# QZ1-boy/FCVSR

Hardware: AMD Instinct MI355X
Metric: SR frames/sec (7-frame window, 4x 180x320->720x1280) + PSNR vs ref (higher is better)
Workload: dtype bf16

## Files before the change

fcvsr_amd/csrc/feat_extract.hip:

```cpp
#include <type_traits>
#include "common.h"
#include "mfma_util.h"
#include "u8.h"

namespace fcvsr {

constexpr int kFePix = 128;
constexpr int kFeK = 64;
constexpr int kFeLD = kFeK + 8;
constexpr int kFeERow = 64 + 4;
constexpr int kFeMaxBlk = 16;

struct FeatArgs {
  View x;
  const float* tab;
  int B, H, W, cin;
  const uint16_t* w;
  const float* bias;
  int n_blk;
  void* dst[kFeMaxBlk];
  long long dsx[kFeMaxBlk];
  int dch[kFeMaxBlk];
};

template <bool DSTBF, int CIN, int SRC = kSrcF32>
__global__ __launch_bounds__(256, 3) void feat_extract_kernel(FeatArgs a) {
  extern __shared__ __align__(16) unsigned char lds[];
  uint16_t* A_s = reinterpret_cast<uint16_t*>(lds);
  const int tid = threadIdx.x;
  const int lane = tid & 63, wave = tid >> 6;
  const int r = lane & 31, h = lane >> 5;
  float* E_s = reinterpret_cast<float*>(lds + kFePix * kFeLD * 2) + wave * (32 * kFeERow);
  const long long npix = (long long)a.B * a.H * a.W;
  const long long flat0 = (long long)blockIdx.x * kFePix;
  float* tab_s = reinterpret_cast<float*>(lds + kFePix * kFeLD * 2);
  static_assert((kPeak10 + 1) * 4 <= 4 * 32 * kFeERow * 4, "the table must fit into the epilogue tile");
  if constexpr (SRC == kSrcU8) {
    tab_s[tid] = a.tab[tid];
    __syncthreads();
  } else if constexpr (SRC == kSrcU16) {
    reinterpret_cast<float4*>(tab_s)[tid] = reinterpret_cast<const float4*>(a.tab)[tid];
    __syncthreads();
  }

  {
    const int pl = tid & (kFePix - 1), half = tid >> 7;
    const long long p = flat0 + pl;
    const bool pok = p < npix;
    const long long pc = pok ? p : npix - 1;
    const int xx = (int)(pc % a.W);
    const int yy = (int)((pc / a.W) % a.H);
    const int b = (int)(pc / ((long long)a.W * a.H));
    const float* xb = a.x.p + (long long)b * a.x.sb;
    const uint8_t* xb8 = reinterpret_cast<const uint8_t*>(a.x.p) + (long long)b * a.x.sb;
    const uint16_t* xb16 = reinterpret_cast<const uint16_t*>(a.x.p) + (long long)b * a.x.sb;
    const int sy = (int)a.x.sy, sx = (int)a.x.sx, sc = (int)a.x.sc;
    float f[32];
    auto gather = [&](auto koff) {
      constexpr int K0 = decltype(koff)::value;
#pragma unroll
      for (int j = 0; j < 32; ++j) {
        constexpr int dummy = 0; (void)dummy;
        const int k = K0 + j;
        const int tap = k / CIN, c = k - tap * CIN;
        const int iy = yy + tap / 3 - 1, ix = xx + tap % 3 - 1;
        const bool in = pok && k < 9 * CIN && iy >= 0 && iy < a.H && ix >= 0 && ix < a.W;
        const int iyc = iy < 0 ? 0 : (iy > a.H - 1 ? a.H - 1 : iy), ixc = ix < 0 ? 0 : (ix > a.W - 1 ? a.W - 1 : ix);
        const int off = iyc * sy + ixc * sx + (k < 9 * CIN ? c : 0) * sc;
        float v;
        if constexpr (SRC == kSrcU8) v = tab_s[xb8[off]];
        else if constexpr (SRC == kSrcU16) v = sample_value<kPeak10>(tab_s, xb16[off]);
        else v = xb[off];
        f[j] = in ? v : 0.f;
      }
    };
    if (half == 0) gather(std::integral_constant<int, 0>{});
    else gather(std::integral_constant<int, 32>{});
    uint4* d = reinterpret_cast<uint4*>(A_s + pl * kFeLD + half * 32);
#pragma unroll
    for (int q = 0; q < 4; ++q) {
      typedef __attribute__((ext_vector_type(8))) _Float16 h8;
      const h8 pk = {(_Float16)f[8 * q], (_Float16)f[8 * q + 1], (_Float16)f[8 * q + 2], (_Float16)f[8 * q + 3],
                     (_Float16)f[8 * q + 4], (_Float16)f[8 * q + 5], (_Float16)f[8 * q + 6], (_Float16)f[8 * q + 7]};
      d[q] = __builtin_bit_cast(uint4, pk);
    }
  }
  __syncthreads();

  uint4 pf[4];
#pragma unroll
  for (int kk = 0; kk < 4; ++kk) pf[kk] = *reinterpret_cast<const uint4*>(A_s + (wave * 32 + r) * kFeLD + kk * 16 + h * 8);

  uint4 wf[2][4];
#define FCVSR_FE_LOADW(BLK)                                                                                   \
  _Pragma("unroll") for (int nf = 0; nf < 2; ++nf) _Pragma("unroll") for (int kk = 0; kk < 4; ++kk)             \
      wf[nf][kk] = *reinterpret_cast<const uint4*>(a.w + ((long long)(BLK) * 64 + nf * 32 + r) * kFeK + kk * 16 + h * 8)
  FCVSR_FE_LOADW(0);
  const int co = lane & 7, psub = lane >> 3;
  for (int blk = 0; blk < a.n_blk; ++blk) {
    f32x16_t acc[2];
#pragma unroll
    for (int nf = 0; nf < 2; ++nf) {
#pragma unroll
      for (int i = 0; i < 16; ++i) acc[nf][i] = 0.f;
#pragma unroll
      for (int kk = 0; kk < 4; ++kk) acc[nf] = mfma<false>(wf[nf][kk], pf[kk], acc[nf]);
    }
    if (blk + 1 < a.n_blk) FCVSR_FE_LOADW(blk + 1);
#pragma unroll
    for (int nf = 0; nf < 2; ++nf)
#pragma unroll
      for (int g = 0; g < 4; ++g)
        *reinterpret_cast<float4*>(E_s + r * kFeERow + nf * 32 + 8 * g + 4 * h) =
            make_float4(acc[nf][4 * g], acc[nf][4 * g + 1], acc[nf][4 * g + 2], acc[nf][4 * g + 3]);
    __builtin_amdgcn_wave_barrier();
    float4 b0 = make_float4(0.f, 0.f, 0.f, 0.f), b1 = b0;
    if (a.bias) {
      b0 = *reinterpret_cast<const float4*>(a.bias + blk * 64 + co * 8);
      b1 = *reinterpret_cast<const float4*>(a.bias + blk * 64 + co * 8 + 4);
    }
    uint16_t* dp = reinterpret_cast<uint16_t*>(a.dst[blk]) + a.dch[blk] + co * 8;
    const long long dsx = a.dsx[blk];
#pragma unroll
    for (int j = 0; j < 4; ++j) {
      const int pl = j * 8 + psub;
      const long long p = flat0 + wave * 32 + pl;
      if (p < npix) {
        const float* es = E_s + pl * kFeERow + co * 8;
        const float4 e0 = *reinterpret_cast<const float4*>(es), e1 = *reinterpret_cast<const float4*>(es + 4);
        const float4 x0 = make_float4(e0.x + b0.x, e0.y + b0.y, e0.z + b0.z, e0.w + b0.w);
        const float4 x1 = make_float4(e1.x + b1.x, e1.y + b1.y, e1.z + b1.z, e1.w + b1.w);
        const uint2 lo = cvt4<DSTBF>(x0), hi = cvt4<DSTBF>(x1);
        *reinterpret_cast<uint4*>(dp + p * dsx) = make_uint4(lo.x, lo.y, hi.x, hi.y);
      }
    }
    __builtin_amdgcn_wave_barrier();
  }
#undef FCVSR_FE_LOADW
}

}

using namespace fcvsr;

template <int SRC>
static int feat_extract_launch(const fcvsr_view* x, const float* tab, int B, int H, int W, const void* w, const float* bias, int n_blk,
                               void* const* dst, const int64_t* dst_pix_stride, const int32_t* dst_ch_off, int dst_dtype, void* stream) {
  FCVSR_CHECK_ARG((long long)H * x->sy < (1ll << 31) && 7ll * x->sc < (1ll << 31), "image too large for 32-bit offsets");
  FCVSR_CHECK_ARG(B > 0 && H > 0 && W > 0 && n_blk >= 1 && n_blk <= kFeMaxBlk, "bad sizes");
  FCVSR_CHECK_ARG(dst_dtype == FCVSR_BF16 || dst_dtype == FCVSR_F16, "16-bit destinations");
  FCVSR_CHECK_ARG(((uintptr_t)w % 16) == 0 && (bias == nullptr || ((uintptr_t)bias % 16) == 0), "weights / bias 16-byte aligned");
  FeatArgs a;
  a.x = to_view(*x); a.tab = tab; a.B = B; a.H = H; a.W = W; a.cin = x->c;
  a.w = (const uint16_t*)w; a.bias = bias; a.n_blk = n_blk;

  for (int i = 0; i < kFeMaxBlk; ++i) {
    const int s = i < n_blk ? i : 0;
    FCVSR_CHECK_ARG(dst[s] && ((uintptr_t)dst[s] % 16) == 0 && dst_pix_stride[s] % 8 == 0 && dst_ch_off[s] % 8 == 0 &&
                        dst_ch_off[s] >= 0, "destinations: 16-byte aligned, strides / offsets multiples of 8");
    a.dst[i] = dst[s]; a.dsx[i] = dst_pix_stride[s]; a.dch[i] = dst_ch_off[s];
  }
  const size_t lds = (size_t)kFePix * kFeLD * 2 + 4ull * 32 * kFeERow * 4;
  static DevOnce attr;
  {
    hipError_t e = once_per_device(attr, [&] {
      hipError_t e1 = hipFuncSetAttribute((const void*)feat_extract_kernel<true, 7, SRC>, hipFuncAttributeMaxDynamicSharedMemorySize, (int)lds);
      if (e1 == hipSuccess)
        e1 = hipFuncSetAttribute((const void*)feat_extract_kernel<false, 7, SRC>, hipFuncAttributeMaxDynamicSharedMemorySize, (int)lds);
      return e1;
    });
    if (e != hipSuccess) {
      set_error("fcvsr_feat_extract: %s", hipGetErrorString(e));
      return (int)e;
    }
  }
  const long long npix = (long long)B * H * W;
  dim3 grid(cdiv(npix, kFePix));
  hipStream_t st = (hipStream_t)stream;
  if (dst_dtype == FCVSR_BF16) hipLaunchKernelGGL((feat_extract_kernel<true, 7, SRC>), grid, dim3(256), lds, st, a);
  else hipLaunchKernelGGL((feat_extract_kernel<false, 7, SRC>), grid, dim3(256), lds, st, a);
  FCVSR_LAUNCH_CHECK();
  return 0;
}

extern "C" int fcvsr_feat_extract(const fcvsr_view* x, int B, int H, int W, const void* w, const float* bias, int n_blk,
                                  void* const* dst, const int64_t* dst_pix_stride, const int32_t* dst_ch_off, int dst_dtype,
                                  void* stream) {
  FCVSR_CHECK_ARG(x && x->ptr && w && dst && dst_pix_stride && dst_ch_off, "null argument");
  FCVSR_CHECK_ARG(x->dtype == FCVSR_F32 && x->c == 7, "x: f32, 7 channels (the Y models' frame stack)");
  return feat_extract_launch<kSrcF32>(x, nullptr, B, H, W, w, bias, n_blk, dst, dst_pix_stride, dst_ch_off, dst_dtype, stream);
}

extern "C" int fcvsr_feat_extract_u8(const fcvsr_view* x, const float* tab, int B, int H, int W, const void* w, const float* bias,
                                     int n_blk, void* const* dst, const int64_t* dst_pix_stride, const int32_t* dst_ch_off,
                                     int dst_dtype, void* stream) {
  FCVSR_CHECK_ARG(x && x->ptr && tab && w && dst && dst_pix_stride && dst_ch_off, "null argument");
  FCVSR_CHECK_ARG(x->dtype == FCVSR_U8 && x->c == 7, "x: uint8, 7 channels (the Y models' frame stack)");
  return feat_extract_launch<kSrcU8>(x, tab, B, H, W, w, bias, n_blk, dst, dst_pix_stride, dst_ch_off, dst_dtype, stream);
}

extern "C" int fcvsr_feat_extract_u16(const fcvsr_view* x, const float* tab, int B, int H, int W, const void* w, const float* bias,
                                      int n_blk, void* const* dst, const int64_t* dst_pix_stride, const int32_t* dst_ch_off,
                                      int dst_dtype, void* stream) {
  FCVSR_CHECK_ARG(x && x->ptr && tab && w && dst && dst_pix_stride && dst_ch_off, "null argument");
  FCVSR_CHECK_ARG(x->dtype == FCVSR_U16 && x->c == 7, "x: uint16, 7 channels (the Y models' frame stack)");
  FCVSR_CHECK_ARG(((uintptr_t)x->ptr % 2) == 0 && ((uintptr_t)tab % 16) == 0, "x 2-byte aligned, table 16-byte aligned");
  return feat_extract_launch<kSrcU16>(x, tab, B, H, W, w, bias, n_blk, dst, dst_pix_stride, dst_ch_off, dst_dtype, stream);
}
```

Measured before the change: 913.9.

## Make feature-extract kernel persistent with LDS-resident weights and register epilogue

Turns the feature-extraction conv kernel into a persistent grid sized to resident blocks per CU. Each block loads all weight blocks (XOR-swizzled) and biases into LDS once, then loops over pixel tiles, gathering the next tile's raw inputs while the current tile's MFMAs run. The LDS im2col staging and LDS epilogue transpose are replaced by direct register fragments plus permlane/DPP shuffles for the output stores, and a specialization with n_blk=7 fully unrolls. In exchange it uses more LDS and registers (launch bounds drop to 2 blocks), and depends on the new device_cu_count and occupancy-query helpers.

```diff
diff --git a/fcvsr_amd/csrc/feat_extract.hip b/fcvsr_amd/csrc/feat_extract.hip
--- a/fcvsr_amd/csrc/feat_extract.hip
+++ b/fcvsr_amd/csrc/feat_extract.hip
@@ -7,8 +7,6 @@
 
 constexpr int kFePix = 128;
 constexpr int kFeK = 64;
-constexpr int kFeLD = kFeK + 8;
-constexpr int kFeERow = 64 + 4;
 constexpr int kFeMaxBlk = 16;
 
 struct FeatArgs {
@@ -18,125 +16,181 @@
   const uint16_t* w;
   const float* bias;
   int n_blk;
+  int ntiles;
   void* dst[kFeMaxBlk];
   long long dsx[kFeMaxBlk];
   int dch[kFeMaxBlk];
 };
 
-template <bool DSTBF, int CIN, int SRC = kSrcF32>
-__global__ __launch_bounds__(256, 3) void feat_extract_kernel(FeatArgs a) {
+template <int SRC> constexpr int fe_tab_floats() { return SRC == kSrcU8 ? kPeak8 + 1 : SRC == kSrcU16 ? kPeak10 + 1 : 0; }
+
+template <int SRC>
+static size_t fe_lds_bytes(int n_blk) { return (size_t)n_blk * 64 * (kFeK * 2 + 4) + fe_tab_floats<SRC>() * 4; }
+
+template <int CIN, int SRC>
+__device__ __forceinline__ void fe_gather(const FeatArgs& a, unsigned p, bool pok, int h, unsigned (&raw)[32], unsigned& inm) {
+  const unsigned q = p / (unsigned)a.W;
+  const int xx = (int)(p - q * (unsigned)a.W);
+  const unsigned b = q / (unsigned)a.H;
+  const int yy = (int)(q - b * (unsigned)a.H);
+  const int sy = (int)a.x.sy, sx = (int)a.x.sx, sc = (int)a.x.sc;
+  int tapoff[9];
+  unsigned tapok = 0;
+#pragma unroll
+  for (int tap = 0; tap < 9; ++tap) {
+    const int iy = yy + tap / 3 - 1, ix = xx + tap % 3 - 1;
+    const bool in = pok && iy >= 0 && iy < a.H && ix >= 0 && ix < a.W;
+    const int iyc = iy < 0 ? 0 : (iy > a.H - 1 ? a.H - 1 : iy), ixc = ix < 0 ? 0 : (ix > a.W - 1 ? a.W - 1 : ix);
+    tapoff[tap] = iyc * sy + ixc * sx;
+    tapok |= (in ? 1u : 0u) << tap;
+  }
+  const float* xb = a.x.p + (long long)b * a.x.sb;
+  const uint8_t* xb8 = reinterpret_cast<const uint8_t*>(a.x.p) + (long long)b * a.x.sb;
+  const uint16_t* xb16 = reinterpret_cast<const uint16_t*>(a.x.p) + (long long)b * a.x.sb;
+  inm = 0;
+#pragma unroll
+  for (int j = 0; j < 32; ++j) {
+    const int k0 = 16 * (j >> 3) + (j & 7), k1 = k0 + 8;
+    const bool v0 = k0 < 9 * CIN, v1 = k1 < 9 * CIN;
+    const int tap0 = v0 ? k0 / CIN : 0, c0 = v0 ? k0 % CIN : 0;
+    const int tap1 = v1 ? k1 / CIN : 0, c1 = v1 ? k1 % CIN : 0;
+    const int off = h ? tapoff[tap1] + c1 * sc : tapoff[tap0] + c0 * sc;
+    const unsigned okbit = h ? (v1 ? (tapok >> tap1) & 1u : 0u) : (v0 ? (tapok >> tap0) & 1u : 0u);
+    inm |= okbit << j;
+    if constexpr (SRC == kSrcU8) raw[j] = xb8[off];
+    else if constexpr (SRC == kSrcU16) raw[j] = xb16[off];
+    else raw[j] = __float_as_uint(xb[off]);
+  }
+}
+
+template <bool DSTBF, int CIN, int SRC, int NB>
+__global__ __launch_bounds__(256, 2) void feat_extract_kernel(FeatArgs a) {
   extern __shared__ __align__(16) unsigned char lds[];
-  uint16_t* A_s = reinterpret_cast<uint16_t*>(lds);
   const int tid = threadIdx.x;
   const int lane = tid & 63, wave = tid >> 6;
   const int r = lane & 31, h = lane >> 5;
-  float* E_s = reinterpret_cast<float*>(lds + kFePix * kFeLD * 2) + wave * (32 * kFeERow);
-  const long long npix = (long long)a.B * a.H * a.W;
-  const long long flat0 = (long long)blockIdx.x * kFePix;
-  float* tab_s = reinterpret_cast<float*>(lds + kFePix * kFeLD * 2);
-  static_assert((kPeak10 + 1) * 4 <= 4 * 32 * kFeERow * 4, "the table must fit into the epilogue tile");
-  if constexpr (SRC == kSrcU8) {
-    tab_s[tid] = a.tab[tid];
-    __syncthreads();
-  } else if constexpr (SRC == kSrcU16) {
-    reinterpret_cast<float4*>(tab_s)[tid] = reinterpret_cast<const float4*>(a.tab)[tid];
-    __syncthreads();
-  }
-
-  {
-    const int pl = tid & (kFePix - 1), half = tid >> 7;
-    const long long p = flat0 + pl;
-    const bool pok = p < npix;
-    const long long pc = pok ? p : npix - 1;
-    const int xx = (int)(pc % a.W);
-    const int yy = (int)((pc / a.W) % a.H);
-    const int b = (int)(pc / ((long long)a.W * a.H));
-    const float* xb = a.x.p + (long long)b * a.x.sb;
-    const uint8_t* xb8 = reinterpret_cast<const uint8_t*>(a.x.p) + (long long)b * a.x.sb;
-    const uint16_t* xb16 = reinterpret_cast<const uint16_t*>(a.x.p) + (long long)b * a.x.sb;
-    const int sy = (int)a.x.sy, sx = (int)a.x.sx, sc = (int)a.x.sc;
-    float f[32];
-    auto gather = [&](auto koff) {
-      constexpr int K0 = decltype(koff)::value;
-#pragma unroll
-      for (int j = 0; j < 32; ++j) {
-        constexpr int dummy = 0; (void)dummy;
-        const int k = K0 + j;
-        const int tap = k / CIN, c = k - tap * CIN;
-        const int iy = yy + tap / 3 - 1, ix = xx + tap % 3 - 1;
-        const bool in = pok && k < 9 * CIN && iy >= 0 && iy < a.H && ix >= 0 && ix < a.W;
-        const int iyc = iy < 0 ? 0 : (iy > a.H - 1 ? a.H - 1 : iy), ixc = ix < 0 ? 0 : (ix > a.W - 1 ? a.W - 1 : ix);
-        const int off = iyc * sy + ixc * sx + (k < 9 * CIN ? c : 0) * sc;
+  const int n_blk = NB ? NB : a.n_blk;
+  unsigned char* W_s = lds;
+  float* bias_s = reinterpret_cast<float*>(lds + (size_t)n_blk * 64 * kFeK * 2);
+  float* tab_s = bias_s + n_blk * 64;
+
+  for (int q = tid; q < n_blk * 64 * 8; q += 256) {
+    const int row = q >> 3, c = q & 7;
+    *reinterpret_cast<uint4*>(W_s + row * 128 + ((c ^ ((row >> 1) & 7)) << 4)) = reinterpret_cast<const uint4*>(a.w)[q];
+  }
+  for (int i = tid; i < n_blk * 64; i += 256) bias_s[i] = a.bias ? a.bias[i] : 0.f;
+  if constexpr (SRC != kSrcF32)
+    for (int i = tid; i < fe_tab_floats<SRC>(); i += 256) tab_s[i] = a.tab[i];
+  __syncthreads();
+
+  const int t_begin = blockIdx.x, t_step = gridDim.x;
+  const unsigned npix = (unsigned)a.B * (unsigned)a.H * (unsigned)a.W;
+  const unsigned char* wrow = W_s + r * 128;
+  const int sw = (r >> 1) & 7;
+
+  uint4 pf[4];
+  auto to_fragments = [&](const unsigned (&raw)[32], unsigned inm) {
+#pragma unroll
+    for (int kk = 0; kk < 4; ++kk) {
+      float f[8];
+#pragma unroll
+      for (int jj = 0; jj < 8; ++jj) {
+        const int j = kk * 8 + jj;
         float v;
-        if constexpr (SRC == kSrcU8) v = tab_s[xb8[off]];
-        else if constexpr (SRC == kSrcU16) v = sample_value<kPeak10>(tab_s, xb16[off]);
-        else v = xb[off];
-        f[j] = in ? v : 0.f;
-      }
-    };
-    if (half == 0) gather(std::integral_constant<int, 0>{});
-    else gather(std::integral_constant<int, 32>{});
-    uint4* d = reinterpret_cast<uint4*>(A_s + pl * kFeLD + half * 32);
-#pragma unroll
-    for (int q = 0; q < 4; ++q) {
+        if constexpr (SRC == kSrcU8) v = tab_s[raw[j]];
+        else if constexpr (SRC == kSrcU16) v = sample_value<kPeak10>(tab_s, raw[j]);
+        else v = __uint_as_float(raw[j]);
+        f[jj] = ((inm >> j) & 1u) ? v : 0.f;
+      }
       typedef __attribute__((ext_vector_type(8))) _Float16 h8;
-      const h8 pk = {(_Float16)f[8 * q], (_Float16)f[8 * q + 1], (_Float16)f[8 * q + 2], (_Float16)f[8 * q + 3],
-                     (_Float16)f[8 * q + 4], (_Float16)f[8 * q + 5], (_Float16)f[8 * q + 6], (_Float16)f[8 * q + 7]};
-      d[q] = __builtin_bit_cast(uint4, pk);
-    }
-  }
-  __syncthreads();
-
-  uint4 pf[4];
-#pragma unroll
-  for (int kk = 0; kk < 4; ++kk) pf[kk] = *reinterpret_cast<const uint4*>(A_s + (wave * 32 + r) * kFeLD + kk * 16 + h * 8);
-
-  uint4 wf[2][4];
+      const h8 pk = {(_Float16)f[0], (_Float16)f[1], (_Float16)f[2], (_Float16)f[3],
+                     (_Float16)f[4], (_Float16)f[5], (_Float16)f[6], (_Float16)f[7]};
+      pf[kk] = __builtin_bit_cast(uint4, pk);
+    }
+  };
+  auto gather_tile = [&](int t, unsigned (&raw)[32], unsigned& inm) {
+    const unsigned p = (unsigned)t * kFePix + wave * 32 + r;
+    fe_gather<CIN, SRC>(a, p < npix ? p : npix - 1, p < npix, h, raw, inm);
+  };
+
+  auto tile = [&](int t, auto full_c) {
+    constexpr bool FULL = decltype(full_c)::value;
+    const unsigned p8 = (unsigned)t * kFePix + wave * 32 + (r & 7);
+    unsigned raw[32], inm;
+    if constexpr (FULL) gather_tile(t + t_step, raw, inm);
+
+    uint4 wf[2][4];
 #define FCVSR_FE_LOADW(BLK)                                                                                   \
   _Pragma("unroll") for (int nf = 0; nf < 2; ++nf) _Pragma("unroll") for (int kk = 0; kk < 4; ++kk)             \
-      wf[nf][kk] = *reinterpret_cast<const uint4*>(a.w + ((long long)(BLK) * 64 + nf * 32 + r) * kFeK + kk * 16 + h * 8)
-  FCVSR_FE_LOADW(0);
-  const int co = lane & 7, psub = lane >> 3;
-  for (int blk = 0; blk < a.n_blk; ++blk) {
-    f32x16_t acc[2];
-#pragma unroll
-    for (int nf = 0; nf < 2; ++nf) {
-#pragma unroll
-      for (int i = 0; i < 16; ++i) acc[nf][i] = 0.f;
-#pragma unroll
-      for (int kk = 0; kk < 4; ++kk) acc[nf] = mfma<false>(wf[nf][kk], pf[kk], acc[nf]);
-    }
-    if (blk + 1 < a.n_blk) FCVSR_FE_LOADW(blk + 1);
-#pragma unroll
-    for (int nf = 0; nf < 2; ++nf)
-#pragma unroll
-      for (int g = 0; g < 4; ++g)
-        *reinterpret_cast<float4*>(E_s + r * kFeERow + nf * 32 + 8 * g + 4 * h) =
-            make_float4(acc[nf][4 * g], acc[nf][4 * g + 1], acc[nf][4 * g + 2], acc[nf][4 * g + 3]);
-    __builtin_amdgcn_wave_barrier();
-    float4 b0 = make_float4(0.f, 0.f, 0.f, 0.f), b1 = b0;
-    if (a.bias) {
-      b0 = *reinterpret_cast<const float4*>(a.bias + blk * 64 + co * 8);
-      b1 = *reinterpret_cast<const float4*>(a.bias + blk * 64 + co * 8 + 4);
-    }
-    uint16_t* dp = reinterpret_cast<uint16_t*>(a.dst[blk]) + a.dch[blk] + co * 8;
-    const long long dsx = a.dsx[blk];
-#pragma unroll
-    for (int j = 0; j < 4; ++j) {
-      const int pl = j * 8 + psub;
-      const long long p = flat0 + wave * 32 + pl;
-      if (p < npix) {
-        const float* es = E_s + pl * kFeERow + co * 8;
-        const float4 e0 = *reinterpret_cast<const float4*>(es), e1 = *reinterpret_cast<const float4*>(es + 4);
-        const float4 x0 = make_float4(e0.x + b0.x, e0.y + b0.y, e0.z + b0.z, e0.w + b0.w);
-        const float4 x1 = make_float4(e1.x + b1.x, e1.y + b1.y, e1.z + b1.z, e1.w + b1.w);
-        const uint2 lo = cvt4<DSTBF>(x0), hi = cvt4<DSTBF>(x1);
-        *reinterpret_cast<uint4*>(dp + p * dsx) = make_uint4(lo.x, lo.y, hi.x, hi.y);
-      }
-    }
-    __builtin_amdgcn_wave_barrier();
-  }
+      wf[nf][kk] = *reinterpret_cast<const uint4*>(wrow + (BLK) * 8192 + nf * 4096 + (((2 * kk + h) ^ sw) << 4))
+    FCVSR_FE_LOADW(0);
+#pragma unroll NB ? NB : 1
+    for (int blk = 0; blk < n_blk; ++blk) {
+      f32x16_t acc[2];
+#pragma unroll
+      for (int nf = 0; nf < 2; ++nf) {
+#pragma unroll
+        for (int i = 0; i < 16; ++i) acc[nf][i] = 0.f;
+#pragma unroll
+        for (int kk = 0; kk < 4; ++kk) acc[nf] = mfma<false>(wf[nf][kk], pf[kk], acc[nf]);
+      }
+      if (blk + 1 < n_blk) FCVSR_FE_LOADW(blk + 1);
+      const float* bs = bias_s + blk * 64 + 4 * h;
+      const bool b3 = (r & 8) != 0;
+      uint16_t* dp = reinterpret_cast<uint16_t*>(a.dst[blk]) + a.dch[blk] + (long long)p8 * a.dsx[blk] + 8 * (h + 2 * (r >> 4)) + (b3 ? 32 : 0);
+      const long long d8 = 8 * a.dsx[blk];
+      typedef __attribute__((ext_vector_type(2))) unsigned u2_t;
+      unsigned c16[2][2][4];
+#pragma unroll
+      for (int nf = 0; nf < 2; ++nf) {
+        unsigned ch[2][4];
+#pragma unroll
+        for (int m = 0; m < 2; ++m) {
+          uint2 pk[2];
+#pragma unroll
+          for (int s = 0; s < 2; ++s) {
+            const int g = 2 * m + s;
+            const float4 b = *reinterpret_cast<const float4*>(bs + nf * 32 + 8 * g);
+            const float4 x = make_float4(acc[nf][4 * g] + b.x, acc[nf][4 * g + 1] + b.y, acc[nf][4 * g + 2] + b.z, acc[nf][4 * g + 3] + b.w);
+            pk[s] = cvt4<DSTBF>(x);
+          }
+          const u2_t s0 = __builtin_amdgcn_permlane32_swap(pk[0].x, pk[1].x, false, false);
+          const u2_t s1 = __builtin_amdgcn_permlane32_swap(pk[0].y, pk[1].y, false, false);
+          ch[m][0] = s0.x; ch[m][1] = s1.x; ch[m][2] = s0.y; ch[m][3] = s1.y;
+        }
+#pragma unroll
+        for (int e = 0; e < 4; ++e) {
+          const u2_t x16 = __builtin_amdgcn_permlane16_swap(ch[0][e], ch[1][e], false, false);
+          c16[nf][0][e] = x16.x; c16[nf][1][e] = x16.y;
+        }
+      }
+#pragma unroll
+      for (int s = 0; s < 2; ++s) {
+        unsigned d0[4], d1[4];
+#pragma unroll
+        for (int e = 0; e < 4; ++e) {
+          const unsigned x0 = c16[0][s][e], x1 = c16[1][s][e];
+          const unsigned got = (unsigned)__builtin_amdgcn_update_dpp(0, (int)(b3 ? x0 : x1), 0x128 , 0xf, 0xf, false);
+          d0[e] = b3 ? got : x0;
+          d1[e] = b3 ? x1 : got;
+        }
+        if (FULL || p8 + 16 * s < npix) *reinterpret_cast<uint4*>(dp + 2 * s * d8) = make_uint4(d0[0], d0[1], d0[2], d0[3]);
+        if (FULL || p8 + 16 * s + 8 < npix) *reinterpret_cast<uint4*>(dp + (2 * s + 1) * d8) = make_uint4(d1[0], d1[1], d1[2], d1[3]);
+      }
+    }
 #undef FCVSR_FE_LOADW
+    if constexpr (FULL) to_fragments(raw, inm);
+  };
+
+  {
+    unsigned raw[32], inm;
+    gather_tile(t_begin, raw, inm);
+    to_fragments(raw, inm);
+  }
+  const int n_full = (int)(npix / kFePix);
+  int t = t_begin;
+  for (; t < n_full; t += t_step) tile(t, std::true_type{});
+  if (t < a.ntiles) tile(t, std::false_type{});
 }
 
 }
@@ -148,6 +202,7 @@
                                void* const* dst, const int64_t* dst_pix_stride, const int32_t* dst_ch_off, int dst_dtype, void* stream) {
   FCVSR_CHECK_ARG((long long)H * x->sy < (1ll << 31) && 7ll * x->sc < (1ll << 31), "image too large for 32-bit offsets");
   FCVSR_CHECK_ARG(B > 0 && H > 0 && W > 0 && n_blk >= 1 && n_blk <= kFeMaxBlk, "bad sizes");
+  FCVSR_CHECK_ARG((long long)B * H * W < (1ll << 31) - 2 * kFePix, "more than 2^31 pixels");
   FCVSR_CHECK_ARG(dst_dtype == FCVSR_BF16 || dst_dtype == FCVSR_F16, "16-bit destinations");
   FCVSR_CHECK_ARG(((uintptr_t)w % 16) == 0 && (bias == nullptr || ((uintptr_t)bias % 16) == 0), "weights / bias 16-byte aligned");
   FeatArgs a;
@@ -160,25 +215,42 @@
                         dst_ch_off[s] >= 0, "destinations: 16-byte aligned, strides / offsets multiples of 8");
     a.dst[i] = dst[s]; a.dsx[i] = dst_pix_stride[s]; a.dch[i] = dst_ch_off[s];
   }
-  const size_t lds = (size_t)kFePix * kFeLD * 2 + 4ull * 32 * kFeERow * 4;
+  typedef void (*fe_kernel_t)(FeatArgs);
+  static const fe_kernel_t kernels[2][2] = {{feat_extract_kernel<false, 7, SRC, 0>, feat_extract_kernel<false, 7, SRC, 7>},
+                                            {feat_extract_kernel<true, 7, SRC, 0>, feat_extract_kernel<true, 7, SRC, 7>}};
+  const int bf = dst_dtype == FCVSR_BF16;
+  const fe_kernel_t kern = kernels[bf][n_blk == 7];
+  const size_t lds = fe_lds_bytes<SRC>(n_blk);
   static DevOnce attr;
+  int dev = 0;
   {
     hipError_t e = once_per_device(attr, [&] {
-      hipError_t e1 = hipFuncSetAttribute((const void*)feat_extract_kernel<true, 7, SRC>, hipFuncAttributeMaxDynamicSharedMemorySize, (int)lds);
-      if (e1 == hipSuccess)
-        e1 = hipFuncSetAttribute((const void*)feat_extract_kernel<false, 7, SRC>, hipFuncAttributeMaxDynamicSharedMemorySize, (int)lds);
+      const int most = (int)fe_lds_bytes<SRC>(kFeMaxBlk);
+      hipError_t e1 = hipSuccess;
+      for (int i = 0; i < 4 && e1 == hipSuccess; ++i)
+        e1 = hipFuncSetAttribute((const void*)kernels[i >> 1][i & 1], hipFuncAttributeMaxDynamicSharedMemorySize, most);
       return e1;
-    });
+    }, &dev);
     if (e != hipSuccess) {
       set_error("fcvsr_feat_extract: %s", hipGetErrorString(e));
       return (int)e;
     }
   }
-  const long long npix = (long long)B * H * W;
-  dim3 grid(cdiv(npix, kFePix));
-  hipStream_t st = (hipStream_t)stream;
-  if (dst_dtype == FCVSR_BF16) hipLaunchKernelGGL((feat_extract_kernel<true, 7, SRC>), grid, dim3(256), lds, st, a);
-  else hipLaunchKernelGGL((feat_extract_kernel<false, 7, SRC>), grid, dim3(256), lds, st, a);
+  static int occ[64][2][kFeMaxBlk + 1];
+  int per_cu = __atomic_load_n(&occ[dev][bf][n_blk], __ATOMIC_RELAXED);
+  if (!per_cu) {
+    hipError_t e = hipOccupancyMaxActiveBlocksPerMultiprocessor(&per_cu, (const void*)kern, 256, lds);
+    if (e != hipSuccess || per_cu < 1) {
+      set_error("fcvsr_feat_extract: occupancy query: %s", hipGetErrorString(e));
+      return e != hipSuccess ? (int)e : FCVSR_E_ARG;
+    }
+    __atomic_store_n(&occ[dev][bf][n_blk], per_cu, __ATOMIC_RELAXED);
+  }
+  const int cus = device_cu_count(dev);
+  a.ntiles = cdiv((long long)B * H * W, kFePix);
+  const int resident = (cus > 0 ? cus : 256) * per_cu;
+  dim3 grid(a.ntiles < resident ? a.ntiles : resident);
+  hipLaunchKernelGGL(kern, grid, dim3(256), lds, (hipStream_t)stream, a);
   FCVSR_LAUNCH_CHECK();
   return 0;
 }
```

Result: no change. 921.6, median of 6 (+0.8%).
